# jiangzhengkai/mxdetection

Measured on AMD Instinct MI355X. Metric: images/sec (whole node) Faster R-CNN R50-FPN 3x800x1333, higher is better.
Workload: dtype bf16; 1 GPU; Faster R-CNN ResNet-50-FPN bf16 train step, batch 2/GPU, 3x800x1333 (padded 1344); global_batch=2, parallelism=dp1, frozen=stem+C2, frozen BN folded, optimizer=SGD momentum 0.9 wd 1e-4, launch=hipGraph replay, input=resident, wgrad_side_stream=True, rpn_branch_stream=True, grouped_wgrad=True, filter_prefetch_hints=True, params_trainable=41538304

## Files before the change

### include/mxdet.h

```cpp
#ifndef MXDET_H_
#define MXDET_H_

#include <stddef.h>
#include <stdint.h>

#ifdef __cplusplus
extern "C" {
#endif

#define MXDET_OK 0
#define MXDET_EINVAL (-1)
#define MXDET_ESHAPE (-2)
#define MXDET_EWORKSPACE (-3)
#define MXDET_EHIP (-4)
#define MXDET_ERCCL (-5)

#define MXDET_DTYPE_F32 0
#define MXDET_DTYPE_BF16 1

typedef void* mxdet_stream_t;

const char* mxdet_last_error(void);
const char* mxdet_version(void);

// ... 58 lines not shown
size_t mxdet_atss_assign_workspace_bytes(int32_t N, int64_t A_total, int32_t G_max);
int mxdet_atss_assign(const float* anchors, int64_t A_total, const int64_t* level_offsets , int32_t L,
                      const float* gt_boxes, int32_t N, int32_t G_max, int32_t topk,
                      int32_t* labels, int32_t* matched_gt, float* bbox_targets, float* matched_iou ,
                      void* workspace, size_t workspace_bytes, mxdet_stream_t stream);

int mxdet_proposal_target(const float* rois, const int32_t* num_rois, int32_t rois_stride,
                          const float* gt_boxes, int32_t N, int32_t G_max, int32_t rois_per_image,
                          float fg_fraction, float fg_thresh, float bg_hi, float bg_lo,
                          int32_t num_classes, int32_t class_agnostic,
                          const float* means , const float* stds ,
                          uint32_t seed, uint32_t step, const uint32_t* step_dev,
                          uint32_t image_offset, float* out_rois, int32_t* labels,
                          float* bbox_targets, float* bbox_weights, int32_t* matched_gt,
                          int32_t* num_fg, mxdet_stream_t stream);

int mxdet_fpn_level_map(const float* rois, int64_t R, int32_t lvl_min, int32_t lvl_max,
                        int32_t* levels, mxdet_stream_t stream);
typedef struct {
  int32_t num_levels, lvl_min;
  int32_t H[8], W[8];
  float spatial_scale[8];
  void* feat[8];
} mxdet_feat_pyramid_t;
int mxdet_roi_align_fwd(const mxdet_feat_pyramid_t* f, int32_t N, int32_t C, const float* rois,
                        const int32_t* levels, int64_t R, int32_t PH, int32_t PW,
                        int32_t sampling_ratio, uint16_t* out, mxdet_stream_t stream);
int mxdet_roi_align_bwd(const mxdet_feat_pyramid_t* f, int32_t N, int32_t C, const float* rois,
                        const int32_t* levels, int64_t R, int32_t PH, int32_t PW,
                        int32_t sampling_ratio, const uint16_t* grad_out, mxdet_stream_t stream);
// ... 311 lines not shown
```

### mxdetection_amd/_lib.py

```python
import ctypes as C
import os

_HERE = os.path.dirname(os.path.abspath(__file__))
LIB_PATH = os.environ.get("MXDET_LIB") or os.path.join(_HERE, "libmxdet_hip.so")

c_i32, c_i64, c_u32, c_f32, c_sz, c_vp = C.c_int32, C.c_int64, C.c_uint32, C.c_float, C.c_size_t, C.c_void_p


class PyramidT(C.Structure):
    _fields_ = [
        ("num_levels", c_i32), ("A", c_i32),
        ("H", c_i32 * 8), ("W", c_i32 * 8), ("stride", c_i32 * 8),
        ("cls", c_vp * 8), ("reg", c_vp * 8),
        ("cls_sn", c_i64 * 8), ("cls_sy", c_i64 * 8), ("cls_sx", c_i64 * 8), ("cls_sa", c_i64 * 8),
        ("reg_sn", c_i64 * 8), ("reg_sy", c_i64 * 8), ("reg_sx", c_i64 * 8), ("reg_sc", c_i64 * 8),
        ("dtype", c_i32), ("classes", c_i32),
        ("base_anchors", c_vp * 8),
    ]


class FeatPyramidT(C.Structure):
    _fields_ = [
        ("num_levels", c_i32), ("lvl_min", c_i32),
        ("H", c_i32 * 8), ("W", c_i32 * 8),
# ... 91 lines not shown
    "mxdet_detection_postprocess_soft": (c_i32, [c_vp, c_vp, c_i32, c_i32, c_i32, c_vp, c_vp, c_vp, c_i32, c_i32, c_i32,
                                                 P(c_f32), P(c_f32), c_f32, c_f32, c_i32, c_vp, c_vp, c_vp, c_sz, c_i32,
                                                 c_f32, c_vp]),
    "mxdet_proposal_workspace_bytes": (c_sz, [P(PyramidT), c_i32, c_i32]),
    "mxdet_proposal": (c_i32, [P(PyramidT), c_i32, c_vp, c_i32, c_i32, c_f32, c_f32, c_vp, c_vp, c_vp, c_vp,
                               c_vp, c_sz, c_vp]),
    "mxdet_anchor_target_workspace_bytes": (c_sz, [c_i32, c_i64, c_i32]),
    "mxdet_anchor_target": (c_i32, [c_vp, c_i64, c_vp, c_i32, c_i32, c_vp, c_f32, c_f32, c_f32, c_i32, c_f32,
                                    c_u32, c_u32, c_vp, c_u32, c_vp, c_vp, c_vp, c_vp, c_vp, c_sz, c_vp]),
    "mxdet_atss_assign_workspace_bytes": (c_sz, [c_i32, c_i64, c_i32]),
    "mxdet_atss_assign": (c_i32, [c_vp, c_i64, P(c_i64), c_i32, c_vp, c_i32, c_i32, c_i32, c_vp, c_vp, c_vp, c_vp, c_vp, c_sz,
                                  c_vp]),
    "mxdet_proposal_target": (c_i32, [c_vp, c_vp, c_i32, c_vp, c_i32, c_i32, c_i32, c_f32, c_f32, c_f32, c_f32,
                                      c_i32, c_i32, P(c_f32), P(c_f32), c_u32, c_u32, c_vp, c_u32, c_vp, c_vp, c_vp,
                                      c_vp, c_vp, c_vp, c_vp]),
    "mxdet_fpn_level_map": (c_i32, [c_vp, c_i64, c_i32, c_i32, c_vp, c_vp]),
    "mxdet_roi_align_fwd": (c_i32, [P(FeatPyramidT), c_i32, c_i32, c_vp, c_vp, c_i64, c_i32, c_i32, c_i32, c_vp,
                                    c_vp]),
    "mxdet_roi_align_bwd": (c_i32, [P(FeatPyramidT), c_i32, c_i32, c_vp, c_vp, c_i64, c_i32, c_i32, c_i32, c_vp,
                                    c_vp]),
    "mxdet_roi_align_bwd_gather_workspace_bytes": (c_sz, [P(FeatPyramidT), c_i32, c_i64]),
    "mxdet_roi_align_bwd_gather": (c_i32, [P(FeatPyramidT), c_i32, c_i32, c_vp, c_vp, c_i64, c_i32, c_i32, c_i32, c_vp,
                                           c_i32, c_vp, c_sz, c_vp]),
    "mxdet_roi_align_bwd_gather_prepare": (c_i32, [P(FeatPyramidT), c_i32, c_vp, c_vp, c_i64, c_i32, c_i32, c_i32,
                                                   c_vp, c_sz, c_vp]),
    "mxdet_roi_align_bwd_gather_prepared": (c_i32, [P(FeatPyramidT), c_i32, c_i32, c_vp, c_vp, c_i64, c_i32, c_i32, c_i32,
                                                    c_vp, c_i32, c_vp, c_sz, c_vp]),
    "mxdet_smooth_l1_fwd": (c_i32, [c_vp, c_vp, c_vp, c_i64, c_f32, c_vp, c_vp]),
    "mxdet_smooth_l1_bwd": (c_i32, [c_vp, c_vp, c_vp, c_vp, c_i64, c_f32, c_i32, c_vp, c_vp]),
    "mxdet_loss_workspace_bytes": (c_sz, [c_i64]),
# ... 141 lines not shown
```

### mxdetection_amd/core/bbox.py

```python
import ctypes as C

import torch

from .. import _lib
from .._lib import check, ptr, stream_ptr


def _f32c(t):
    assert t.is_cuda and t.dtype == torch.float32 and t.is_contiguous(), "expected contiguous cuda float32"
    return t


def bbox_overlaps(boxes, query_boxes):
    lib = _lib.load()
    _f32c(boxes), _f32c(query_boxes)
    out = torch.empty((boxes.shape[0], query_boxes.shape[0]), dtype=torch.float32, device=boxes.device)
    check(lib.mxdet_box_iou(ptr(boxes), boxes.shape[0], ptr(query_boxes), query_boxes.shape[0], ptr(out),
                            stream_ptr()), "box_iou")
    return out


def sample_rois(rois, num_rois, gt_boxes, rois_per_image=512, fg_fraction=0.25, fg_thresh=0.5, bg_thresh_hi=0.5,
                bg_thresh_lo=0.0, num_classes=81, class_agnostic=False, bbox_means=(0.0, 0.0, 0.0, 0.0),
                bbox_stds=(0.1, 0.1, 0.2, 0.2), seed=0, step=0, image_offset=0, step_dev=None):
    lib = _lib.load()
    _f32c(rois), _f32c(gt_boxes)
    N, S = rois.shape[0], rois.shape[1]
    G = gt_boxes.shape[1]
    R = rois_per_image
    D = 4 if class_agnostic else 4 * num_classes
    dev = rois.device
    out_rois = torch.empty((N, R, 5), dtype=torch.float32, device=dev)
    labels = torch.empty((N, R), dtype=torch.int32, device=dev)
    tgt = torch.empty((N, R, D), dtype=torch.float32, device=dev)
    wgt = torch.empty((N, R, D), dtype=torch.float32, device=dev)
    matched = torch.empty((N, R), dtype=torch.int32, device=dev)
    num_fg = torch.empty((N,), dtype=torch.int32, device=dev)
    means = (C.c_float * 4)(*bbox_means)
    stds = (C.c_float * 4)(*bbox_stds)
    check(lib.mxdet_proposal_target(ptr(rois), ptr(num_rois), S, ptr(gt_boxes), N, G, R, fg_fraction, fg_thresh,
                                    bg_thresh_hi, bg_thresh_lo, num_classes, int(class_agnostic), means, stds,
                                    seed, step, ptr(step_dev), image_offset, ptr(out_rois), ptr(labels), ptr(tgt), ptr(wgt),
                                    ptr(matched), ptr(num_fg), stream_ptr()), "proposal_target")
    return out_rois, labels, tgt, wgt, matched, num_fg
```

### mxdetection_amd/csrc/boxes.hip

```cpp
#include "common.h"

namespace mxdet {

__global__ void box_iou_kernel(const float4* __restrict__ a, int64_t na, const float4* __restrict__ b,
                               int64_t nb, float* __restrict__ out) {
  int64_t idx = (int64_t)blockIdx.x * blockDim.x + threadIdx.x;
  if (idx >= na * nb) return;
  int64_t i = idx / nb, j = idx - i * nb;
  float4 p = a[i], q = b[j];
  out[idx] = mxdet_iou(p.x, p.y, p.z, p.w, q.x, q.y, q.z, q.w);
}

__global__ void anchors_kernel(const float* __restrict__ base, int A, int H, int W, int stride,
                               float4* __restrict__ out) {
  int64_t idx = (int64_t)blockIdx.x * blockDim.x + threadIdx.x;
  int64_t total = (int64_t)H * W * A;
  if (idx >= total) return;
  int a = (int)(idx % A);
  int64_t cell = idx / A;
  int x = (int)(cell % W), y = (int)(cell / W);
  float sx = (float)(x * stride), sy = (float)(y * stride);
  float4 o;
  o.x = base[a * 4 + 0] + sx;
  o.y = base[a * 4 + 1] + sy;
  o.z = base[a * 4 + 2] + sx;
  o.w = base[a * 4 + 3] + sy;
  out[idx] = o;
}

__global__ void fpn_level_kernel(const float* __restrict__ rois, int64_t R, int lvl_min, int lvl_max,
                                 int32_t* __restrict__ levels) {
  int64_t i = (int64_t)blockIdx.x * blockDim.x + threadIdx.x;
  if (i >= R) return;
  const float* r = rois + i * 5;
  int k = mxdet_fpn_level(r[1], r[2], r[3], r[4]);
  k = k < lvl_min ? lvl_min : (k > lvl_max ? lvl_max : k);
  levels[i] = k;
}

__global__ void __launch_bounds__(64)
nms_mask_kernel(const float4* __restrict__ boxes, const int32_t* __restrict__ counts, int n_max,
                int nwords_max, float thresh, unsigned long long* __restrict__ mask) {
  const int col_blk = blockIdx.x, row_blk = blockIdx.y, b = blockIdx.z;
  if (col_blk < row_blk) return;
  int n = counts[b];
  n = n > n_max ? n_max : n;
  if (row_blk * 64 >= n || col_blk * 64 >= n) return;
  __shared__ float4 cb[64];
  const int t = threadIdx.x;
  const float4* bx = boxes + (int64_t)b * n_max;
  int cj = col_blk * 64 + t;
  if (cj < n) cb[t] = bx[cj];
  __syncthreads();
  int i = row_blk * 64 + t;
  if (i >= n) return;
  float4 r = bx[i];
  int ncol = n - col_blk * 64;
  ncol = ncol > 64 ? 64 : ncol;
  unsigned long long bits = 0;
  for (int j = 0; j < ncol; ++j) {
    int c = col_blk * 64 + j;
    float4 q = cb[j];
    float v = mxdet_iou(r.x, r.y, r.z, r.w, q.x, q.y, q.z, q.w);
    if (c > i && v > thresh) bits |= (1ull << j);
  }
  mask[((int64_t)b * n_max + i) * nwords_max + col_blk] = bits;
}

__device__ __forceinline__ unsigned long long readlane64(unsigned long long v, int lane) {
  unsigned lo = (unsigned)v, hi = (unsigned)(v >> 32);
  lo = (unsigned)__builtin_amdgcn_readlane((int)lo, lane);
  hi = (unsigned)__builtin_amdgcn_readlane((int)hi, lane);
  return ((unsigned long long)hi << 32) | lo;
}

__global__ void __launch_bounds__(64)
nms_scan_kernel(const unsigned long long* __restrict__ mask, const int32_t* __restrict__ counts,
                const uint8_t* __restrict__ invalid, int n_max, int nwords_max, int max_keep,
                int32_t* __restrict__ keep_idx, int32_t* __restrict__ num_keep) {
// ... 47 lines not shown
  }
  int excl = incl - cnt;
  int total = __shfl(incl, 63);
  unsigned long long kb = mykeep;
  int pos = excl;
  while (kb) {
    int bb = __ffsll((long long)kb) - 1;
    kb &= kb - 1;
    if (pos < max_keep) keep_idx[(int64_t)b * n_max + pos] = lane * 64 + bb;
    ++pos;
  }
  if (lane == 0) num_keep[b] = total < max_keep ? total : max_keep;
}

template <int NW>
__global__ void __launch_bounds__(64)
nms_scan_rows_kernel(const unsigned long long* __restrict__ mask, const int32_t* __restrict__ counts,
                     const uint8_t* __restrict__ invalid, int n_max, int nwords_max, int max_keep,
                     int32_t* __restrict__ keep_idx, int32_t* __restrict__ num_keep) {
  __shared__ unsigned long long rows[2][64][NW + 1];
  const int b = blockIdx.x, lane = threadIdx.x;
  int n = counts[b];
  n = n > n_max ? n_max : n;
  n = __builtin_amdgcn_readfirstlane(n);
  const int nw = (n + 63) >> 6;
  const unsigned long long* m = mask + (int64_t)b * n_max * NW;
  unsigned long long myrem = 0ull;
  for (int w = 0; w < nw; ++w) {
    int idx = w * 64 + lane;
    bool bad = (idx >= n) || (invalid != nullptr && invalid[(int64_t)b * n_max + idx] != 0);
    unsigned long long bm = __ballot(bad);
    if (lane == w) myrem = bm;
  }
  unsigned long long nxt[NW];
  auto load_row = [&](unsigned long long (&r)[NW], int w) {
    const unsigned long long* bp = m + (int64_t)(w * 64) * NW + lane;
#pragma unroll
    for (int k = 0; k < NW; ++k) r[k] = bp[k * 64];
  };
  auto stage = [&](const unsigned long long (&r)[NW], int buf, int w) {
    unsigned long long* dst = &rows[buf][lane >> 5][lane & 31];
#pragma unroll
    for (int k = 0; k < NW; ++k) dst[k * 2 * (NW + 1)] = r[k];
  };
  load_row(nxt, 0);
  stage(nxt, 0, 0);
  __syncthreads();
  const int myword = lane < NW ? lane : 0;
  unsigned long long mykeep = 0;
  int buf = 0;
  for (int w = 0; w < nw; ++w) {
#ifndef NMS_ABL_NOLOAD
    if (w + 1 < nw) load_row(nxt, w + 1);
#endif
    const unsigned long long diag = rows[buf][lane][w];
    unsigned long long c = readlane64(myrem, w);
#ifndef NMS_ABL_NOCHAIN
#pragma unroll
    for (int bb = 0; bb < 64; ++bb) {
      unsigned long long d = readlane64(diag, bb);
      c |= ((c >> bb) & 1ull) ? 0ull : d;
    }
#else
    c |= readlane64(diag, 0);
#endif
    const unsigned long long keepbits = ~c;
    if (lane == w) mykeep = keepbits;
    const unsigned klo = __builtin_amdgcn_readfirstlane((unsigned)keepbits);
    const unsigned khi = __builtin_amdgcn_readfirstlane((unsigned)(keepbits >> 32));
    unsigned long long acc = 0ull;
#ifndef NMS_ABL_NOOR
#pragma unroll
#else
    if (klo == 0x12345u)
#endif
    for (int ch = 0; ch < 8; ++ch) {
      const unsigned bits = ((ch < 4 ? klo : khi) >> (8 * (ch & 3))) & 0xffu;
      if (bits == 0u) continue;
      unsigned long long v[8];
#pragma unroll
      for (int t = 0; t < 8; ++t) v[t] = rows[buf][8 * ch + t][myword];
#pragma unroll
      for (int t = 0; t < 8; ++t) acc |= ((bits >> t) & 1u) ? v[t] : 0ull;
    }
    if (lane > w && lane < nw) myrem |= acc;
    if (w + 1 < nw) stage(nxt, buf ^ 1, w + 1);
    __syncthreads();
    buf ^= 1;
  }
  int cnt = __popcll(mykeep);
  int incl = cnt;
  for (int off = 1; off < 64; off <<= 1) {
    int v = __shfl_up(incl, off);
    if (lane >= off) incl += v;
  }
  int excl = incl - cnt;
  int total = __shfl(incl, 63);
  unsigned long long kb = mykeep;
  int pos = excl;
  while (kb) {
    int bb = __ffsll((long long)kb) - 1;
    kb &= kb - 1;
    if (pos < max_keep) keep_idx[(int64_t)b * n_max + pos] = lane * 64 + bb;
    ++pos;
// ... 28 lines not shown
                     as_stream(stream), base_anchors, A, H, W, stride, (float4*)out);
  return check_launch("generate_anchors");
}

extern "C" int mxdet_fpn_level_map(const float* rois, int64_t R, int32_t lvl_min, int32_t lvl_max,
                                   int32_t* levels, mxdet_stream_t stream) {
  clear_error();
  MXDET_REQUIRE(R >= 0 && lvl_min <= lvl_max, MXDET_ESHAPE, "fpn_level_map: bad arguments");
  if (R == 0) return MXDET_OK;
  MXDET_REQUIRE(rois && levels, MXDET_EINVAL, "fpn_level_map: null pointer");
  hipLaunchKernelGGL(fpn_level_kernel, dim3((unsigned)ceil_div<int64_t>(R, 256)), dim3(256), 0,
                     as_stream(stream), rois, R, lvl_min, lvl_max, levels);
  return check_launch("fpn_level_map");
}

extern "C" size_t mxdet_nms_batched_workspace_bytes(int32_t B, int32_t n_max) {
  if (B <= 0 || n_max <= 0) return 0;
  size_t nwords = (size_t)(n_max + 63) / 64;
  if (nwords <= 32) nwords = 32;
  return ((size_t)B * n_max + 64) * nwords * sizeof(unsigned long long);
}

extern "C" int mxdet_nms_batched(const float* boxes, const int32_t* counts, const uint8_t* invalid,
                                 int32_t B, int32_t n_max, float thresh, int32_t max_keep,
                                 int32_t* keep_idx, int32_t* num_keep, void* workspace,
                                 size_t workspace_bytes, mxdet_stream_t stream) {
  clear_error();
  MXDET_REQUIRE(B >= 0 && n_max >= 0, MXDET_ESHAPE, "nms_batched: negative size");
  if (B == 0) return MXDET_OK;
  MXDET_REQUIRE(n_max <= 4096, MXDET_ESHAPE, "nms_batched: n_max %d > 4096 unsupported", n_max);
  MXDET_REQUIRE(counts && num_keep, MXDET_EINVAL, "nms_batched: null pointer");
  if (n_max == 0) {
    hipError_t e = zero_async(num_keep, sizeof(int32_t) * B, as_stream(stream));
    MXDET_REQUIRE(e == hipSuccess, MXDET_EHIP, "nms_batched: memset failed");
    return MXDET_OK;
  }
  MXDET_REQUIRE(boxes && keep_idx, MXDET_EINVAL, "nms_batched: null pointer");
  size_t need = mxdet_nms_batched_workspace_bytes(B, n_max);
  MXDET_REQUIRE(workspace && workspace_bytes >= need, MXDET_EWORKSPACE,
                "nms_batched: workspace %zu < %zu", workspace_bytes, need);
  int nwords = (n_max + 63) / 64;
  const int pitch = nwords <= 32 ? 32 : nwords;
  hipLaunchKernelGGL(nms_mask_kernel, dim3(nwords, nwords, B), dim3(64), 0, as_stream(stream),
                     (const float4*)boxes, counts, n_max, pitch, thresh,
                     (unsigned long long*)workspace);
  if (nwords <= 32)
    hipLaunchKernelGGL(nms_scan_rows_kernel<32>, dim3(B), dim3(64), 0, as_stream(stream),
                       (const unsigned long long*)workspace, counts, invalid, n_max, nwords,
                       max_keep < 0 ? 0 : max_keep, keep_idx, num_keep);
  else
    hipLaunchKernelGGL(nms_scan_kernel, dim3(B), dim3(64), 0, as_stream(stream),
                       (const unsigned long long*)workspace, counts, invalid, n_max, nwords,
                       max_keep < 0 ? 0 : max_keep, keep_idx, num_keep);
  return check_launch("nms_batched");
}
```

### mxdetection_amd/csrc/targets.hip

```cpp
#include "common.h"
#include "select.h"

namespace mxdet {

__global__ void __launch_bounds__(256)
anchor_iou_kernel(const float4* __restrict__ anchors, long long A_total, const float* __restrict__ gt,
                  int G_max, const float* __restrict__ im_info, float allowed_border,
                  float* __restrict__ max_iou, int32_t* __restrict__ argmax,
                  unsigned* __restrict__ gt_max) {
  extern __shared__ __attribute__((aligned(16))) unsigned char smem_raw[];
  float* sg = (float*)smem_raw;
  unsigned* sgm = (unsigned*)(sg + G_max * 5);
  const int n = blockIdx.y;
  for (int i = threadIdx.x; i < G_max * 5; i += blockDim.x) sg[i] = gt[(long long)n * G_max * 5 + i];
  for (int i = threadIdx.x; i < G_max; i += blockDim.x) sgm[i] = 0u;
  __syncthreads();
  long long a = (long long)blockIdx.x * blockDim.x + threadIdx.x;
  if (a < A_total) {
    float4 b = anchors[a];
    float im_h = im_info[n * 3 + 0], im_w = im_info[n * 3 + 1];
    bool inside = (b.x >= -allowed_border) && (b.y >= -allowed_border) &&
                  (b.z < im_w + allowed_border) && (b.w < im_h + allowed_border);
    float best = -1.0f;
    int bi = -1;
// ... 196 lines not shown
    float o[4];
    mxdet_encode(b.x, b.y, b.z, b.w, q[0], q[1], q[2], q[3], o);
    t = make_float4(o[0], o[1], o[2], o[3]);
  }
  targets[idx] = t;
}

__global__ void __launch_bounds__(1024)
proposal_target_kernel(const float* __restrict__ rois, const int32_t* __restrict__ num_rois,
                       int rois_stride, const float* __restrict__ gt, int G_max, int R, int max_fg,
                       float fg_thresh, float bg_hi, float bg_lo, int num_classes, int class_agnostic,
                       float4 means, float4 stds, unsigned seed, unsigned step,
                       const unsigned* __restrict__ step_dev, unsigned image_offset,
                       float* __restrict__ out_rois, int32_t* __restrict__ labels,
                       float* __restrict__ bbox_targets, float* __restrict__ bbox_weights,
                       int32_t* __restrict__ matched_gt, int32_t* __restrict__ num_fg_out) {
  extern __shared__ __attribute__((aligned(16))) unsigned char smem_raw[];
  const int ncap = rois_stride + G_max;
  float* sg = (float*)smem_raw;
  int* vg = (int*)(sg + G_max * 5);
  short* cgt = (short*)(vg + G_max);
  signed char* cstate = (signed char*)(cgt + ((ncap + 7) & ~7));
  __shared__ SelectSmem sm;
  __shared__ int n_valid_gt, cnt_bg;
  const int n = blockIdx.x;
  const unsigned image = image_offset + (unsigned)n;
  if (step_dev) step = *step_dev;
  for (int i = threadIdx.x; i < G_max * 5; i += blockDim.x) sg[i] = gt[(long long)n * G_max * 5 + i];
  if (threadIdx.x == 0) cnt_bg = 0;
  __syncthreads();
  if (threadIdx.x == 0) {
// ... 49 lines not shown
  const int want_bg = (R - nfg) > 0 ? (R - nfg) : 0;
  if (threadIdx.x == 0) cnt_bg = sel_b.n_cand < want_bg ? sel_b.n_cand : want_bg;
  for (int i = threadIdx.x; i < nc; i += blockDim.x) {
    unsigned kv;
    if (cstate[i] == 1) { kfg(i, kv); if (sel_f.chosen(kv, (unsigned)i)) cstate[i] = 3; }
    else if (cstate[i] == 2) { kbg(i, kv); if (sel_b.chosen(kv, (unsigned)i)) cstate[i] = 4; }
  }
  __syncthreads();
  const int nbg = cnt_bg;
  const int reg_dim = class_agnostic ? 4 : 4 * num_classes;
  float* orois = out_rois + (long long)n * R * 5;
  int32_t* olab = labels + (long long)n * R;
  float* otgt = bbox_targets + (long long)n * R * reg_dim;
  float* owgt = bbox_weights + (long long)n * R * reg_dim;
  int32_t* omg = matched_gt + (long long)n * R;
  for (int s = nfg + nbg + threadIdx.x; s < R; s += blockDim.x) {
    float* r = orois + (long long)s * 5;
    r[0] = (float)n; r[1] = 0.f; r[2] = 0.f; r[3] = 0.f; r[4] = 0.f;
    olab[s] = -1;
    omg[s] = -1;
  }
  __syncthreads();
  int base_fg = 0, base_bg = 0;
  for (int base = 0; base < nc; base += blockDim.x) {
    int i = base + threadIdx.x;
    signed char st = (i < nc) ? cstate[i] : 0;
    int tf, tb;
    int rf = block_excl_count(st == 3, sm.scratch, &tf);
    int rbk = block_excl_count(st == 4, sm.scratch, &tb);
    if (st == 3 || st == 4) {
      int slot = (st == 3) ? (base_fg + rf) : (nfg + base_bg + rbk);
      float b[4];
      cand_box(i, b);
      float* r = orois + (long long)slot * 5;
      r[0] = (float)n; r[1] = b[0]; r[2] = b[1]; r[3] = b[2]; r[4] = b[3];
      int g = cgt[i];
      omg[slot] = g;
      if (st == 3) {
        const float* q = sg + g * 5;
        int cls = (int)q[4];
        olab[slot] = cls;
        float o[4];
        mxdet_encode(b[0], b[1], b[2], b[3], q[0], q[1], q[2], q[3], o);
        int c0 = class_agnostic ? 0 : 4 * cls;
        float* t = otgt + (long long)slot * reg_dim + c0;
        float* w = owgt + (long long)slot * reg_dim + c0;
        t[0] = (o[0] - means.x) / stds.x;
        t[1] = (o[1] - means.y) / stds.y;
        t[2] = (o[2] - means.z) / stds.z;
        t[3] = (o[3] - means.w) / stds.w;
// ... 81 lines not shown
  hipLaunchKernelGGL(anchor_nogt_kernel, grid, dim3(256), 0, s, (const float4*)anchors,
                     (long long)A_total, gt_boxes, G_max, im_info, allowed_border, seed, step, step_dev,
                     image_offset, labels, miou, w.keys, cl);
  if (batch_size > 0) {
    int max_fg = (int)(fg_fraction * (float)batch_size);
    hipLaunchKernelGGL(anchor_sample_kernel, dim3(N), dim3(1024), 0, s, (long long)A_total,
                       batch_size, max_fg, (const int32_t*)labels, (const unsigned*)w.keys, cl, w.sel);
  }
  hipLaunchKernelGGL(anchor_encode_kernel, grid, dim3(256), 0, s, (const float4*)anchors,
                     (long long)A_total, gt_boxes, G_max, labels, amax, (const unsigned*)w.keys,
                     batch_size > 0 ? (const AnchorSel*)w.sel : (const AnchorSel*)nullptr,
                     (float4*)bbox_targets);
  return check_launch("anchor_target");
}

extern "C" int mxdet_proposal_target(const float* rois, const int32_t* num_rois, int32_t rois_stride,
                                     const float* gt_boxes, int32_t N, int32_t G_max,
                                     int32_t rois_per_image, float fg_fraction, float fg_thresh,
                                     float bg_hi, float bg_lo, int32_t num_classes,
                                     int32_t class_agnostic, const float* means, const float* stds,
                                     uint32_t seed, uint32_t step, const uint32_t* step_dev,
                                     uint32_t image_offset, float* out_rois, int32_t* labels,
                                     float* bbox_targets,
                                     float* bbox_weights, int32_t* matched_gt, int32_t* num_fg,
                                     mxdet_stream_t stream) {
  clear_error();
  MXDET_REQUIRE(N > 0 && rois_stride > 0 && G_max > 0 && rois_per_image > 0 && num_classes > 0,
                MXDET_ESHAPE, "proposal_target: bad sizes");
  MXDET_REQUIRE(rois && num_rois && gt_boxes && means && stds && out_rois && labels && bbox_targets &&
                    bbox_weights && matched_gt && num_fg,
                MXDET_EINVAL, "proposal_target: null pointer");
  MXDET_REQUIRE(G_max <= 1024 && rois_stride <= 16384, MXDET_ESHAPE, "proposal_target: too large");
  int ncap = rois_stride + G_max;
  size_t lds = (size_t)G_max * 5 * 4 + (size_t)G_max * 4 + (size_t)((ncap + 7) & ~7) * 2 +
               (size_t)((ncap + 15) & ~15);
  MXDET_REQUIRE(lds <= 120 * 1024, MXDET_ESHAPE, "proposal_target: LDS budget exceeded");
  int max_fg = (int)(fg_fraction * (float)rois_per_image);
  float4 m = make_float4(means[0], means[1], means[2], means[3]);
  float4 sd = make_float4(stds[0], stds[1], stds[2], stds[3]);
  {
    const size_t reg_dim = class_agnostic ? 4 : 4 * (size_t)num_classes;
    const size_t bytes = (size_t)N * rois_per_image * reg_dim * sizeof(float);
    hipError_t e = zero_async(bbox_targets, bytes, as_stream(stream));
    if (e == hipSuccess) e = zero_async(bbox_weights, bytes, as_stream(stream));
    MXDET_REQUIRE(e == hipSuccess, MXDET_EHIP, "proposal_target: zero fill failed");
  }
  hipLaunchKernelGGL(proposal_target_kernel, dim3(N), dim3(1024), lds, as_stream(stream), rois,
                     num_rois, rois_stride, gt_boxes, G_max, rois_per_image, max_fg, fg_thresh, bg_hi,
                     bg_lo, num_classes, class_agnostic, m, sd, seed, step, step_dev, image_offset, out_rois,
                     labels, bbox_targets, bbox_weights, matched_gt, num_fg);
  return check_launch("proposal_target");
}
```

### mxdetection_amd/models/bbox_heads/convfc_bbox_head.py

```python
import os

import torch

from ...core import bbox as B_
from ...core import loss as L_
from ...ops import dense
from ..utils.layers import ConvLayer, GroupNormLayer, cached_buf


class BBoxHead:
    def __init__(self, in_features, arena, ws, device, gen, num_classes=81, fc_dim=1024, rois_per_image=512,
                 fg_fraction=0.25, fg_thresh=0.5, bg_hi=0.5, bg_lo=0.0, stds=(0.1, 0.1, 0.2, 0.2), sigma=1.0,
                 seed=99, reg_loss="smooth_l1", reg_loss_weight=1.0):
        L_.check_reg_loss(reg_loss, reg_loss_weight)
        self.reg_loss, self.reg_loss_weight = reg_loss, float(reg_loss_weight)
        kw = dict(arena=arena, ws=ws, device=device, gen=gen)
        self.nc = num_classes
        self.reg_dim = 4 * num_classes
        self.ld = (num_classes + self.reg_dim + 63) // 64 * 64
        self.fc_out = ConvLayer("bbox.fc_out", fc_dim, self.ld, 1, init_std=0.01, cout_real=num_classes + self.reg_dim, **kw)
        self._build_trunk(in_features, fc_dim, kw)
        self.fc_out.fc_in_hwc = ()
        self.R, self.fg_fraction, self.fg_thresh, self.bg_hi, self.bg_lo = rois_per_image, fg_fraction, fg_thresh, bg_hi, bg_lo
        self.stds, self.sigma, self.seed, self.device = stds, sigma, seed, device
# ... 13 lines not shown

    def norm_layers(self):
        return []

    def _buf(self, key, shape, dtype=torch.bfloat16, zero=False):
        return cached_buf(self.bufs, key, shape, dtype, self.device, zero)

    def plan(self, N):
        R = N * self.R
        self.fc1.plan((R, 1, 1, self.in_features))
        self.fc2.plan((R, 1, 1, self.fc_dim))
        self.fc_out.plan((R, 1, 1, self.fc_dim))
        self.loss = torch.zeros((2,), dtype=torch.float32, device=self.device)
        self.loss_ws = L_.loss_workspace(R, self.device)

    def sample(self, rois, num_rois, gt_boxes, step, image_offset, step_dev=None):
        out = B_.sample_rois(rois, num_rois, gt_boxes, self.R, self.fg_fraction, self.fg_thresh, self.bg_hi, self.bg_lo,
                             self.nc, False, (0.0, 0.0, 0.0, 0.0), self.stds, self.seed, step, image_offset, step_dev)
        self.rois, self.labels, self.tgt, self.wgt, self.matched, self.num_fg = out
        self.gt_boxes = gt_boxes
        return self.rois.view(-1, 5)

    def forward(self, pooled):
        R = pooled.shape[0]
        self.x = pooled.view(R, 1, 1, -1)
        ks = self.fc1_ksplit if (R * self.fc_dim) % (64 * 64 * 8) == 0 and R % 64 == 0 else 1
        if ks > 1:
            need = 4 * ks * R * self.fc_dim
            ws = self._buf("fc1_ws", (need,), dtype=torch.uint8)
            self.h1 = dense.conv2d_forward_splitk(self.x, self.fc1.w_bf16, self.fc1.bias_f32, None, True, ks,
                                                  self._buf("h1", (R, 1, 1, self.fc_dim)), ws)
        else:
            self.h1 = self.fc1.forward(self.x, relu=True, out=self._buf("h1", (R, 1, 1, self.fc_dim)))
        self.h2 = self.fc2.forward(self.h1, relu=True, out=self._buf("h2", (R, 1, 1, self.fc_dim)))
# ... 102 lines not shown
```

### mxdetection_amd/models/faster_rcnn.py

```python
import torch

from ..core.loss import check_reg_loss
from .backbones import ResNet
from .bbox_heads import BBoxHead, ConvFCBBoxHead
from .mask_heads import FCNMaskHead
from .necks import FPN
from .roi_extractors import DeformRoIExtractor, FPNRoIExtractor
from .rpn_heads import RPNHead
from .utils.detector import DetectorBase
from .utils.layers import Workspace


def check_head_options(bbox_head, head_norm, gn_groups, with_mask):
    if bbox_head not in ("2fc", "4conv1fc"):
        raise ValueError("bbox_head must be '2fc' or '4conv1fc' (got %r)" % (bbox_head,))
    if head_norm not in ("none", "gn"):
        raise ValueError("head_norm must be 'none' or 'gn' (got %r)" % (head_norm,))
    if head_norm == "gn":
        if bbox_head == "2fc" and not with_mask:
            raise ValueError("head_norm='gn' with nothing to normalise: the 2fc box head has no convolutions and there "
                             "is no mask head")
        g = gn_groups
        if not isinstance(g, int) or isinstance(g, bool) or g <= 0 or 256 % g or (256 // g) % 8:
            raise ValueError("gn_groups = %r does not divide 256 channels into groups of a multiple of 8" % (g,))
# ... 82 lines not shown
        N, _, H, W = image.shape
        self.plan(N, H, W, gt_boxes.shape[1])
        early = self.branch is not None
        if early:
            with self._branch_ctx():
                self.rpn_head.assign_targets(gt_boxes, im_info, step, image_offset, step_dev)
        C = self.backbone.forward(image)
        P = self.neck.forward(C)
        self.rpn_head.forward(P)
        defer_rpn = (self.roi_bwd_gather and self.ws.side is not None and self.ws_rpn.grouping and self.ws.grouping
                     and self._bucket_here(0))
        with self._branch_ctx():
            rpn_loss = self.rpn_head.loss_and_grad(gt_boxes, im_info, step, image_offset, step_dev=step_dev, assigned=early)
            self.rpn_head.backward(self.dP, [False] * 5, flush=not defer_rpn)
        rois, _, _, num_rois = self.rpn_head.get_proposals(im_info)
        rois_s = self.bbox_head.sample(rois, num_rois, gt_boxes, step, image_offset, step_dev)
        pooled = self.roi_extractor.forward(P, rois_s, prepare_gather=self.roi_bwd_gather)
        self.bbox_head.forward(pooled)
        rcnn_loss = self.bbox_head.loss_and_grad()
        mask_loss = None
        if self.with_mask:
            mrois = self.mask_head.select_rois(self.bbox_head)
            self.mask_head.targets(gt_masks)
            mpooled = self.mask_roi_extractor.forward(P, mrois, prepare_gather=self.roi_bwd_gather)
            self.mask_head.forward(mpooled)
            mask_loss = self.mask_head.loss_and_grad()
        if self.with_mask:
            d_mpooled = self.mask_head.backward()
        d_pooled = self.bbox_head.backward()
        if self.roi_bwd_gather:
            self._join_branch()
            lo = 0
# ... 56 lines not shown
```

### mxdetection_amd/models/roi_extractors/fpn_roi_extractor.py

```python
import torch

from ...ops import dense
from ...ops.roi_align import (fpn_level_map, roi_align_backward, roi_align_backward_gather,
                              roi_align_backward_gather_prepare, roi_align_backward_gather_workspace, roi_align_forward)


class FPNRoIExtractor:
    def __init__(self, strides, pooled=(7, 7), sampling_ratio=2, lvl_min=2, device="cuda"):
        self.scales = [1.0 / s for s in strides]
        self.pooled, self.sr, self.lvl_min = pooled, sampling_ratio, lvl_min
        self.lvl_max = lvl_min + len(strides) - 1
        self.device = device
        self.out = None
        self.outs = {}
        self.dacc = None
        self.gather_ws = {}
        self.prepared = None

    def forward(self, feats, rois, prepare_gather=False):
        self.feats, self.rois = feats[:len(self.scales)], rois
        self.levels = fpn_level_map(rois, self.lvl_min, self.lvl_max)
        R, C = rois.shape[0], feats[0].shape[3]
        self.out = self.outs.setdefault((R, C), None)
        if self.out is None:
            self.out = torch.empty((R, self.pooled[0], self.pooled[1], C), dtype=torch.bfloat16, device=self.device)
            self.outs[(R, C)] = self.out
        self.prepared = None
        if prepare_gather:
            key = (R,) + tuple(tuple(f.shape[:3]) for f in self.feats)
            ws = self.gather_ws.get(key)
            if ws is None:
                ws = self.gather_ws[key] = roi_align_backward_gather_workspace(self.feats, self.scales, R, self.lvl_min)
            roi_align_backward_gather_prepare(self.feats, self.scales, rois, self.levels, self.pooled, self.sr,
                                              self.lvl_min, ws)
            self.prepared = ws
        return roi_align_forward(self.feats, self.scales, rois, self.levels, self.pooled, self.sr, self.lvl_min, self.out)
# ... 37 lines not shown
```

### mxdetection_amd/ops/nms.py

```python
import torch

from .. import _lib
from .._lib import check, ptr, stream_ptr


def nms_batched(boxes, counts, thresh, max_keep=None, invalid=None):
    lib = _lib.load()
    B, n = boxes.shape[0], boxes.shape[1]
    dev = boxes.device
    keep = torch.full((B, max(n, 1)), -1, dtype=torch.int32, device=dev)
    num = torch.zeros((B,), dtype=torch.int32, device=dev)
    ws_bytes = lib.mxdet_nms_batched_workspace_bytes(B, n)
    ws = torch.empty((max(ws_bytes, 8),), dtype=torch.uint8, device=dev)
    check(lib.mxdet_nms_batched(ptr(boxes), ptr(counts), ptr(invalid), B, n, thresh,
                                n if max_keep is None else max_keep, ptr(keep), ptr(num), ptr(ws), ws_bytes,
                                stream_ptr()), "nms_batched")
    return keep, num


SOFT_NMS_METHODS = {"hard": 0, "linear": 1, "gaussian": 2}


def soft_nms_method(name):
    if name not in SOFT_NMS_METHODS:
        raise ValueError("nms_method %r: expected one of %s" % (name, sorted(SOFT_NMS_METHODS)))
    return SOFT_NMS_METHODS[name]


# ... 12 lines not shown
```

Baseline: 480.0 images/sec.

## Restructure batched NMS mask/scan kernels and fuse FPN level mapping into ROI sampling

The NMS mask kernel now launches only the upper-triangular block pairs, packing four column blocks per 256-thread workgroup, and also records within-block column suppression bits. The row-scan kernel becomes a 256-thread kernel that resolves each 64-box word with an iterative ballot fixed point, spreads the OR-reduction over four waves and prefetches three words ahead. Separately, proposal-target sampling now also writes FPN level indices, so the ROI extractor no longer launches its own level-map kernel. nms_batched also accepts a caller-supplied workspace. These changes aim to cut kernel count and serial latency in the RPN/ROI stage, but add more complex synchronisation and a fixed-point loop that can take up to 64 rounds.

```diff
diff --git a/include/mxdet.h b/include/mxdet.h
--- a/include/mxdet.h
+++ b/include/mxdet.h
@@ -96,6 +96,16 @@
                           uint32_t image_offset, float* out_rois, int32_t* labels,
                           float* bbox_targets, float* bbox_weights, int32_t* matched_gt,
                           int32_t* num_fg, mxdet_stream_t stream);
+int mxdet_proposal_target_levels(const float* rois, const int32_t* num_rois, int32_t rois_stride,
+                                 const float* gt_boxes, int32_t N, int32_t G_max, int32_t rois_per_image,
+                                 float fg_fraction, float fg_thresh, float bg_hi, float bg_lo,
+                                 int32_t num_classes, int32_t class_agnostic,
+                                 const float* means , const float* stds ,
+                                 uint32_t seed, uint32_t step, const uint32_t* step_dev,
+                                 uint32_t image_offset, float* out_rois, int32_t* labels,
+                                 float* bbox_targets, float* bbox_weights, int32_t* matched_gt,
+                                 int32_t* num_fg, int32_t lvl_min, int32_t lvl_max, int32_t* levels,
+                                 mxdet_stream_t stream);
 
 int mxdet_fpn_level_map(const float* rois, int64_t R, int32_t lvl_min, int32_t lvl_max,
                         int32_t* levels, mxdet_stream_t stream);
diff --git a/mxdetection_amd/_lib.py b/mxdetection_amd/_lib.py
--- a/mxdetection_amd/_lib.py
+++ b/mxdetection_amd/_lib.py
@@ -129,6 +129,9 @@
     "mxdet_proposal_target": (c_i32, [c_vp, c_vp, c_i32, c_vp, c_i32, c_i32, c_i32, c_f32, c_f32, c_f32, c_f32,
                                       c_i32, c_i32, P(c_f32), P(c_f32), c_u32, c_u32, c_vp, c_u32, c_vp, c_vp, c_vp,
                                       c_vp, c_vp, c_vp, c_vp]),
+    "mxdet_proposal_target_levels": (c_i32, [c_vp, c_vp, c_i32, c_vp, c_i32, c_i32, c_i32, c_f32, c_f32, c_f32, c_f32,
+                                             c_i32, c_i32, P(c_f32), P(c_f32), c_u32, c_u32, c_vp, c_u32, c_vp, c_vp, c_vp,
+                                             c_vp, c_vp, c_vp, c_i32, c_i32, c_vp, c_vp]),
     "mxdet_fpn_level_map": (c_i32, [c_vp, c_i64, c_i32, c_i32, c_vp, c_vp]),
     "mxdet_roi_align_fwd": (c_i32, [P(FeatPyramidT), c_i32, c_i32, c_vp, c_vp, c_i64, c_i32, c_i32, c_i32, c_vp,
                                     c_vp]),
diff --git a/mxdetection_amd/core/bbox.py b/mxdetection_amd/core/bbox.py
--- a/mxdetection_amd/core/bbox.py
+++ b/mxdetection_amd/core/bbox.py
@@ -22,7 +22,7 @@
 
 def sample_rois(rois, num_rois, gt_boxes, rois_per_image=512, fg_fraction=0.25, fg_thresh=0.5, bg_thresh_hi=0.5,
                 bg_thresh_lo=0.0, num_classes=81, class_agnostic=False, bbox_means=(0.0, 0.0, 0.0, 0.0),
-                bbox_stds=(0.1, 0.1, 0.2, 0.2), seed=0, step=0, image_offset=0, step_dev=None):
+                bbox_stds=(0.1, 0.1, 0.2, 0.2), seed=0, step=0, image_offset=0, step_dev=None, fpn_levels=None):
     lib = _lib.load()
     _f32c(rois), _f32c(gt_boxes)
     N, S = rois.shape[0], rois.shape[1]
@@ -38,8 +38,13 @@
     num_fg = torch.empty((N,), dtype=torch.int32, device=dev)
     means = (C.c_float * 4)(*bbox_means)
     stds = (C.c_float * 4)(*bbox_stds)
-    check(lib.mxdet_proposal_target(ptr(rois), ptr(num_rois), S, ptr(gt_boxes), N, G, R, fg_fraction, fg_thresh,
-                                    bg_thresh_hi, bg_thresh_lo, num_classes, int(class_agnostic), means, stds,
-                                    seed, step, ptr(step_dev), image_offset, ptr(out_rois), ptr(labels), ptr(tgt), ptr(wgt),
-                                    ptr(matched), ptr(num_fg), stream_ptr()), "proposal_target")
-    return out_rois, labels, tgt, wgt, matched, num_fg
+    args = (ptr(rois), ptr(num_rois), S, ptr(gt_boxes), N, G, R, fg_fraction, fg_thresh, bg_thresh_hi, bg_thresh_lo,
+            num_classes, int(class_agnostic), means, stds, seed, step, ptr(step_dev), image_offset, ptr(out_rois),
+            ptr(labels), ptr(tgt), ptr(wgt), ptr(matched), ptr(num_fg))
+    if fpn_levels is None:
+        check(lib.mxdet_proposal_target(*args, stream_ptr()), "proposal_target")
+        return out_rois, labels, tgt, wgt, matched, num_fg
+    levels = torch.empty((N, R), dtype=torch.int32, device=dev)
+    check(lib.mxdet_proposal_target_levels(*args, fpn_levels[0], fpn_levels[1], ptr(levels), stream_ptr()),
+          "proposal_target_levels")
+    return out_rois, labels, tgt, wgt, matched, num_fg, levels
diff --git a/mxdetection_amd/csrc/boxes.hip b/mxdetection_amd/csrc/boxes.hip
--- a/mxdetection_amd/csrc/boxes.hip
+++ b/mxdetection_amd/csrc/boxes.hip
@@ -38,31 +38,51 @@
   levels[i] = k;
 }
 
-__global__ void __launch_bounds__(64)
-nms_mask_kernel(const float4* __restrict__ boxes, const int32_t* __restrict__ counts, int n_max,
-                int nwords_max, float thresh, unsigned long long* __restrict__ mask) {
-  const int col_blk = blockIdx.x, row_blk = blockIdx.y, b = blockIdx.z;
-  if (col_blk < row_blk) return;
+__global__ void __launch_bounds__(256)
+nms_mask_kernel(const float4* __restrict__ boxes, const int32_t* __restrict__ counts, int n_max, int nwords,
+                int nwords_max, float thresh, unsigned long long* __restrict__ mask,
+                unsigned long long* __restrict__ cols) {
+  __shared__ float4 cb[4][64];
+  const int b = blockIdx.y, wave = threadIdx.x >> 6, t = threadIdx.x & 63;
+  int row_blk = 0, rest = blockIdx.x;
+  for (int r = 0; r < nwords; ++r) {
+    const int groups = (nwords - r + 3) >> 2;
+    if (rest < groups) { row_blk = r; break; }
+    rest -= groups;
+  }
+  const int col_blk = row_blk + rest * 4 + wave;
   int n = counts[b];
   n = n > n_max ? n_max : n;
-  if (row_blk * 64 >= n || col_blk * 64 >= n) return;
-  __shared__ float4 cb[64];
-  const int t = threadIdx.x;
+  if (row_blk * 64 >= n) return;
+  const bool live = col_blk < nwords && col_blk * 64 < n;
   const float4* bx = boxes + (int64_t)b * n_max;
   int cj = col_blk * 64 + t;
-  if (cj < n) cb[t] = bx[cj];
+  cb[wave][t] = (live && cj < n) ? bx[cj] : make_float4(0.f, 0.f, 0.f, 0.f);
   __syncthreads();
   int i = row_blk * 64 + t;
-  if (i >= n) return;
+  if (!live || i >= n) return;
   float4 r = bx[i];
   int ncol = n - col_blk * 64;
   ncol = ncol > 64 ? 64 : ncol;
   unsigned long long bits = 0;
-  for (int j = 0; j < ncol; ++j) {
-    int c = col_blk * 64 + j;
-    float4 q = cb[j];
-    float v = mxdet_iou(r.x, r.y, r.z, r.w, q.x, q.y, q.z, q.w);
-    if (c > i && v > thresh) bits |= (1ull << j);
+  if (col_blk != row_blk) {
+    for (int j = 0; j < ncol; ++j) {
+      float4 q = cb[wave][j];
+      float v = mxdet_iou(r.x, r.y, r.z, r.w, q.x, q.y, q.z, q.w);
+      if (v > thresh) bits |= (1ull << j);
+    }
+  } else {
+    unsigned long long cbits = 0;
+    for (int j = 0; j < ncol; ++j) {
+      float4 q = cb[wave][j];
+      const bool up = j > t;
+      float4 p0 = up ? r : q, p1 = up ? q : r;
+      float v = mxdet_iou(p0.x, p0.y, p0.z, p0.w, p1.x, p1.y, p1.z, p1.w);
+      if (j != t && v > thresh) {
+        if (up) bits |= (1ull << j); else cbits |= (1ull << j);
+      }
+    }
+    cols[(int64_t)b * n_max + i] = cbits;
   }
   mask[((int64_t)b * n_max + i) * nwords_max + col_blk] = bits;
 }
@@ -140,80 +160,109 @@
 }
 
 template <int NW>
-__global__ void __launch_bounds__(64)
-nms_scan_rows_kernel(const unsigned long long* __restrict__ mask, const int32_t* __restrict__ counts,
-                     const uint8_t* __restrict__ invalid, int n_max, int nwords_max, int max_keep,
+__global__ void __launch_bounds__(256)
+nms_scan_rows_kernel(const unsigned long long* __restrict__ mask, const unsigned long long* __restrict__ cols,
+                     const int32_t* __restrict__ counts, const uint8_t* __restrict__ invalid, int n_max, int max_keep,
                      int32_t* __restrict__ keep_idx, int32_t* __restrict__ num_keep) {
+  static_assert(NW == 32, "the thread -> (row group, word) maps below assume 32 words");
+  constexpr int kGroups = 256 / NW;
+  constexpr int kRowsPer = 64 / kGroups;
+  constexpr int kLoads = 64 * NW / 256;
   __shared__ unsigned long long rows[2][64][NW + 1];
-  const int b = blockIdx.x, lane = threadIdx.x;
+  __shared__ unsigned long long part[2][kGroups][NW];
+  __shared__ unsigned long long rem0[NW];
+  __shared__ unsigned long long colw[2][64];
+  const int b = blockIdx.x, tid = threadIdx.x, lane = tid & 63, wave = tid >> 6;
   int n = counts[b];
   n = n > n_max ? n_max : n;
   n = __builtin_amdgcn_readfirstlane(n);
   const int nw = (n + 63) >> 6;
   const unsigned long long* m = mask + (int64_t)b * n_max * NW;
-  unsigned long long myrem = 0ull;
-  for (int w = 0; w < nw; ++w) {
-    int idx = w * 64 + lane;
-    bool bad = (idx >= n) || (invalid != nullptr && invalid[(int64_t)b * n_max + idx] != 0);
-    unsigned long long bm = __ballot(bad);
-    if (lane == w) myrem = bm;
-  }
-  unsigned long long nxt[NW];
-  auto load_row = [&](unsigned long long (&r)[NW], int w) {
-    const unsigned long long* bp = m + (int64_t)(w * 64) * NW + lane;
-#pragma unroll
-    for (int k = 0; k < NW; ++k) r[k] = bp[k * 64];
+  const unsigned long long* cl = cols + (int64_t)b * n_max;
+  {
+    bool bad[NW / 4];
+#pragma unroll
+    for (int k = 0; k < NW / 4; ++k) {
+      int idx = (wave + 4 * k) * 64 + lane;
+      bad[k] = (idx >= n) || (invalid != nullptr && invalid[(int64_t)b * n_max + idx] != 0);
+    }
+#pragma unroll
+    for (int k = 0; k < NW / 4; ++k) {
+      unsigned long long bm = __ballot(bad[k]);
+      if (lane == 0) rem0[wave + 4 * k] = bm;
+    }
+  }
+  struct Fetch { unsigned long long r[kLoads], col; };
+  auto load_rows = [&](Fetch& f, int w) {
+    if (w >= nw) return;
+    const unsigned long long* bp = m + (int64_t)(w * 64) * NW + tid;
+#pragma unroll
+    for (int k = 0; k < kLoads; ++k) f.r[k] = bp[k * 256];
+    const int idx = w * 64 + lane;
+    f.col = idx < n ? cl[idx] : 0ull;
   };
-  auto stage = [&](const unsigned long long (&r)[NW], int buf, int w) {
-    unsigned long long* dst = &rows[buf][lane >> 5][lane & 31];
-#pragma unroll
-    for (int k = 0; k < NW; ++k) dst[k * 2 * (NW + 1)] = r[k];
+  auto stage = [&](const Fetch& f, int buf) {
+    unsigned long long* dst = &rows[buf][tid / NW][tid % NW];
+#pragma unroll
+    for (int k = 0; k < kLoads; ++k) dst[k * kGroups * (NW + 1)] = f.r[k];
+    if (wave == 0) colw[buf][lane] = f.col;
   };
-  load_row(nxt, 0);
-  stage(nxt, 0, 0);
+  Fetch fa, fb, fc;
+  load_rows(fa, 0);
+  load_rows(fb, 1);
+  load_rows(fc, 2);
+  if (nw > 0) stage(fa, 0);
   __syncthreads();
-  const int myword = lane < NW ? lane : 0;
+  const int myword = lane % NW;
+  const int grp = tid / NW;
+  unsigned long long myrem = rem0[myword];
   unsigned long long mykeep = 0;
-  int buf = 0;
-  for (int w = 0; w < nw; ++w) {
+  auto word = [&](int w, Fetch& ld, const Fetch& st) {
+    const int buf = w & 1;
 #ifndef NMS_ABL_NOLOAD
-    if (w + 1 < nw) load_row(nxt, w + 1);
+    load_rows(ld, w + 3);
 #endif
-    const unsigned long long diag = rows[buf][lane][w];
-    unsigned long long c = readlane64(myrem, w);
+    const unsigned long long col = colw[buf][lane];
+    const unsigned long long removed = readlane64(myrem, w);
+    const bool alive = !((removed >> lane) & 1ull);
+    unsigned long long K = ~removed;
 #ifndef NMS_ABL_NOCHAIN
-#pragma unroll
-    for (int bb = 0; bb < 64; ++bb) {
-      unsigned long long d = readlane64(diag, bb);
-      c |= ((c >> bb) & 1ull) ? 0ull : d;
+    for (int round = 0; round < 64; ++round) {
+      const unsigned long long K1 = __ballot(alive && (col & K) == 0ull);
+      if (K1 == K) break;
+      K = K1;
     }
 #else
-    c |= readlane64(diag, 0);
+    K = __ballot(alive && (col & K) == 0ull);
 #endif
-    const unsigned long long keepbits = ~c;
+    const unsigned long long keepbits = K;
     if (lane == w) mykeep = keepbits;
-    const unsigned klo = __builtin_amdgcn_readfirstlane((unsigned)keepbits);
-    const unsigned khi = __builtin_amdgcn_readfirstlane((unsigned)(keepbits >> 32));
     unsigned long long acc = 0ull;
-#ifndef NMS_ABL_NOOR
-#pragma unroll
-#else
-    if (klo == 0x12345u)
+#ifdef NMS_ABL_NOOR
+    if (keepbits == 0x12345ull)
 #endif
-    for (int ch = 0; ch < 8; ++ch) {
-      const unsigned bits = ((ch < 4 ? klo : khi) >> (8 * (ch & 3))) & 0xffu;
-      if (bits == 0u) continue;
-      unsigned long long v[8];
-#pragma unroll
-      for (int t = 0; t < 8; ++t) v[t] = rows[buf][8 * ch + t][myword];
-#pragma unroll
-      for (int t = 0; t < 8; ++t) acc |= ((bits >> t) & 1u) ? v[t] : 0ull;
-    }
-    if (lane > w && lane < nw) myrem |= acc;
-    if (w + 1 < nw) stage(nxt, buf ^ 1, w + 1);
+    {
+      const unsigned kb = (unsigned)(keepbits >> (kRowsPer * grp)) & ((1u << kRowsPer) - 1u);
+      unsigned long long v[kRowsPer];
+#pragma unroll
+      for (int t = 0; t < kRowsPer; ++t) v[t] = rows[buf][kRowsPer * grp + t][myword];
+#pragma unroll
+      for (int t = 0; t < kRowsPer; ++t) acc |= ((kb >> t) & 1u) ? v[t] : 0ull;
+    }
+    part[buf][grp][myword] = acc;
+    if (w + 1 < nw) stage(st, buf ^ 1);
     __syncthreads();
-    buf ^= 1;
-  }
+    unsigned long long sum = 0ull;
+#pragma unroll
+    for (int g = 0; g < kGroups; ++g) sum |= part[buf][g][myword];
+    if (myword > w && myword < nw) myrem |= sum;
+  };
+  for (int w = 0; w < nw; w += 3) {
+    word(w, fa, fb);
+    if (w + 1 < nw) word(w + 1, fb, fc);
+    if (w + 2 < nw) word(w + 2, fc, fa);
+  }
+  if (wave != 0) return;
   int cnt = __popcll(mykeep);
   int incl = cnt;
   for (int off = 1; off < 64; off <<= 1) {
@@ -272,11 +321,15 @@
   return check_launch("fpn_level_map");
 }
 
-extern "C" size_t mxdet_nms_batched_workspace_bytes(int32_t B, int32_t n_max) {
-  if (B <= 0 || n_max <= 0) return 0;
+static size_t nms_mask_bytes(int32_t B, int32_t n_max) {
   size_t nwords = (size_t)(n_max + 63) / 64;
   if (nwords <= 32) nwords = 32;
   return ((size_t)B * n_max + 64) * nwords * sizeof(unsigned long long);
+}
+
+extern "C" size_t mxdet_nms_batched_workspace_bytes(int32_t B, int32_t n_max) {
+  if (B <= 0 || n_max <= 0) return 0;
+  return nms_mask_bytes(B, n_max) + (size_t)B * n_max * sizeof(unsigned long long);
 }
 
 extern "C" int mxdet_nms_batched(const float* boxes, const int32_t* counts, const uint8_t* invalid,
@@ -299,12 +352,15 @@
                 "nms_batched: workspace %zu < %zu", workspace_bytes, need);
   int nwords = (n_max + 63) / 64;
   const int pitch = nwords <= 32 ? 32 : nwords;
-  hipLaunchKernelGGL(nms_mask_kernel, dim3(nwords, nwords, B), dim3(64), 0, as_stream(stream),
-                     (const float4*)boxes, counts, n_max, pitch, thresh,
-                     (unsigned long long*)workspace);
+  unsigned long long* cols = (unsigned long long*)((char*)workspace + nms_mask_bytes(B, n_max));
+  int tri = 0;
+  for (int r = 0; r < nwords; ++r) tri += (nwords - r + 3) / 4;
+  hipLaunchKernelGGL(nms_mask_kernel, dim3(tri, B), dim3(256), 0, as_stream(stream),
+                     (const float4*)boxes, counts, n_max, nwords, pitch, thresh,
+                     (unsigned long long*)workspace, cols);
   if (nwords <= 32)
-    hipLaunchKernelGGL(nms_scan_rows_kernel<32>, dim3(B), dim3(64), 0, as_stream(stream),
-                       (const unsigned long long*)workspace, counts, invalid, n_max, nwords,
+    hipLaunchKernelGGL(nms_scan_rows_kernel<32>, dim3(B), dim3(256), 0, as_stream(stream),
+                       (const unsigned long long*)workspace, (const unsigned long long*)cols, counts, invalid, n_max,
                        max_keep < 0 ? 0 : max_keep, keep_idx, num_keep);
   else
     hipLaunchKernelGGL(nms_scan_kernel, dim3(B), dim3(64), 0, as_stream(stream),
diff --git a/mxdetection_amd/csrc/targets.hip b/mxdetection_amd/csrc/targets.hip
--- a/mxdetection_amd/csrc/targets.hip
+++ b/mxdetection_amd/csrc/targets.hip
@@ -234,7 +234,8 @@
                        const unsigned* __restrict__ step_dev, unsigned image_offset,
                        float* __restrict__ out_rois, int32_t* __restrict__ labels,
                        float* __restrict__ bbox_targets, float* __restrict__ bbox_weights,
-                       int32_t* __restrict__ matched_gt, int32_t* __restrict__ num_fg_out) {
+                       int32_t* __restrict__ matched_gt, int32_t* __restrict__ num_fg_out, int lvl_min, int lvl_max,
+                       int32_t* __restrict__ levels) {
   extern __shared__ __attribute__((aligned(16))) unsigned char smem_raw[];
   const int ncap = rois_stride + G_max;
   float* sg = (float*)smem_raw;
@@ -314,11 +315,17 @@
   float* otgt = bbox_targets + (long long)n * R * reg_dim;
   float* owgt = bbox_weights + (long long)n * R * reg_dim;
   int32_t* omg = matched_gt + (long long)n * R;
+  int32_t* olvl = levels ? levels + (long long)n * R : nullptr;
+  auto fpn_lvl = [&](float x1, float y1, float x2, float y2) {
+    int k = mxdet_fpn_level(x1, y1, x2, y2);
+    return k < lvl_min ? lvl_min : (k > lvl_max ? lvl_max : k);
+  };
   for (int s = nfg + nbg + threadIdx.x; s < R; s += blockDim.x) {
     float* r = orois + (long long)s * 5;
     r[0] = (float)n; r[1] = 0.f; r[2] = 0.f; r[3] = 0.f; r[4] = 0.f;
     olab[s] = -1;
     omg[s] = -1;
+    if (olvl) olvl[s] = fpn_lvl(0.f, 0.f, 0.f, 0.f);
   }
   __syncthreads();
   int base_fg = 0, base_bg = 0;
@@ -334,6 +341,7 @@
       cand_box(i, b);
       float* r = orois + (long long)slot * 5;
       r[0] = (float)n; r[1] = b[0]; r[2] = b[1]; r[3] = b[2]; r[4] = b[3];
+      if (olvl) olvl[slot] = fpn_lvl(b[0], b[1], b[2], b[3]);
       int g = cgt[i];
       omg[slot] = g;
       if (st == 3) {
@@ -445,16 +453,16 @@
   return check_launch("anchor_target");
 }
 
-extern "C" int mxdet_proposal_target(const float* rois, const int32_t* num_rois, int32_t rois_stride,
-                                     const float* gt_boxes, int32_t N, int32_t G_max,
-                                     int32_t rois_per_image, float fg_fraction, float fg_thresh,
-                                     float bg_hi, float bg_lo, int32_t num_classes,
-                                     int32_t class_agnostic, const float* means, const float* stds,
-                                     uint32_t seed, uint32_t step, const uint32_t* step_dev,
-                                     uint32_t image_offset, float* out_rois, int32_t* labels,
-                                     float* bbox_targets,
-                                     float* bbox_weights, int32_t* matched_gt, int32_t* num_fg,
-                                     mxdet_stream_t stream) {
+static int proposal_target_impl(const float* rois, const int32_t* num_rois, int32_t rois_stride,
+                                const float* gt_boxes, int32_t N, int32_t G_max,
+                                int32_t rois_per_image, float fg_fraction, float fg_thresh,
+                                float bg_hi, float bg_lo, int32_t num_classes,
+                                int32_t class_agnostic, const float* means, const float* stds,
+                                uint32_t seed, uint32_t step, const uint32_t* step_dev,
+                                uint32_t image_offset, float* out_rois, int32_t* labels,
+                                float* bbox_targets,
+                                float* bbox_weights, int32_t* matched_gt, int32_t* num_fg,
+                                int32_t lvl_min, int32_t lvl_max, int32_t* levels, mxdet_stream_t stream) {
   clear_error();
   MXDET_REQUIRE(N > 0 && rois_stride > 0 && G_max > 0 && rois_per_image > 0 && num_classes > 0,
                 MXDET_ESHAPE, "proposal_target: bad sizes");
@@ -479,6 +487,40 @@
   hipLaunchKernelGGL(proposal_target_kernel, dim3(N), dim3(1024), lds, as_stream(stream), rois,
                      num_rois, rois_stride, gt_boxes, G_max, rois_per_image, max_fg, fg_thresh, bg_hi,
                      bg_lo, num_classes, class_agnostic, m, sd, seed, step, step_dev, image_offset, out_rois,
-                     labels, bbox_targets, bbox_weights, matched_gt, num_fg);
+                     labels, bbox_targets, bbox_weights, matched_gt, num_fg, lvl_min, lvl_max, levels);
   return check_launch("proposal_target");
 }
+
+extern "C" int mxdet_proposal_target(const float* rois, const int32_t* num_rois, int32_t rois_stride,
+                                     const float* gt_boxes, int32_t N, int32_t G_max,
+                                     int32_t rois_per_image, float fg_fraction, float fg_thresh,
+                                     float bg_hi, float bg_lo, int32_t num_classes,
+                                     int32_t class_agnostic, const float* means, const float* stds,
+                                     uint32_t seed, uint32_t step, const uint32_t* step_dev,
+                                     uint32_t image_offset, float* out_rois, int32_t* labels,
+                                     float* bbox_targets,
+                                     float* bbox_weights, int32_t* matched_gt, int32_t* num_fg,
+                                     mxdet_stream_t stream) {
+  return proposal_target_impl(rois, num_rois, rois_stride, gt_boxes, N, G_max, rois_per_image, fg_fraction, fg_thresh,
+                              bg_hi, bg_lo, num_classes, class_agnostic, means, stds, seed, step, step_dev, image_offset,
+                              out_rois, labels, bbox_targets, bbox_weights, matched_gt, num_fg, 0, 0, nullptr, stream);
+}
+
+extern "C" int mxdet_proposal_target_levels(const float* rois, const int32_t* num_rois, int32_t rois_stride,
+                                            const float* gt_boxes, int32_t N, int32_t G_max,
+                                            int32_t rois_per_image, float fg_fraction, float fg_thresh,
+                                            float bg_hi, float bg_lo, int32_t num_classes,
+                                            int32_t class_agnostic, const float* means, const float* stds,
+                                            uint32_t seed, uint32_t step, const uint32_t* step_dev,
+                                            uint32_t image_offset, float* out_rois, int32_t* labels,
+                                            float* bbox_targets, float* bbox_weights, int32_t* matched_gt,
+                                            int32_t* num_fg, int32_t lvl_min, int32_t lvl_max, int32_t* levels,
+                                            mxdet_stream_t stream) {
+  clear_error();
+  MXDET_REQUIRE(levels != nullptr, MXDET_EINVAL, "proposal_target_levels: null levels");
+  MXDET_REQUIRE(lvl_min <= lvl_max, MXDET_ESHAPE, "proposal_target_levels: lvl_min %d > lvl_max %d", lvl_min, lvl_max);
+  return proposal_target_impl(rois, num_rois, rois_stride, gt_boxes, N, G_max, rois_per_image, fg_fraction, fg_thresh,
+                              bg_hi, bg_lo, num_classes, class_agnostic, means, stds, seed, step, step_dev, image_offset,
+                              out_rois, labels, bbox_targets, bbox_weights, matched_gt, num_fg, lvl_min, lvl_max, levels,
+                              stream);
+}
diff --git a/mxdetection_amd/models/bbox_heads/convfc_bbox_head.py b/mxdetection_amd/models/bbox_heads/convfc_bbox_head.py
--- a/mxdetection_amd/models/bbox_heads/convfc_bbox_head.py
+++ b/mxdetection_amd/models/bbox_heads/convfc_bbox_head.py
@@ -51,10 +51,12 @@
         self.loss = torch.zeros((2,), dtype=torch.float32, device=self.device)
         self.loss_ws = L_.loss_workspace(R, self.device)
 
-    def sample(self, rois, num_rois, gt_boxes, step, image_offset, step_dev=None):
+    def sample(self, rois, num_rois, gt_boxes, step, image_offset, step_dev=None, fpn_levels=None):
         out = B_.sample_rois(rois, num_rois, gt_boxes, self.R, self.fg_fraction, self.fg_thresh, self.bg_hi, self.bg_lo,
-                             self.nc, False, (0.0, 0.0, 0.0, 0.0), self.stds, self.seed, step, image_offset, step_dev)
-        self.rois, self.labels, self.tgt, self.wgt, self.matched, self.num_fg = out
+                             self.nc, False, (0.0, 0.0, 0.0, 0.0), self.stds, self.seed, step, image_offset, step_dev,
+                             fpn_levels=fpn_levels)
+        self.rois, self.labels, self.tgt, self.wgt, self.matched, self.num_fg = out[:6]
+        self.roi_levels = out[6].view(-1) if fpn_levels is not None else None
         self.gt_boxes = gt_boxes
         return self.rois.view(-1, 5)
 
diff --git a/mxdetection_amd/models/faster_rcnn.py b/mxdetection_amd/models/faster_rcnn.py
--- a/mxdetection_amd/models/faster_rcnn.py
+++ b/mxdetection_amd/models/faster_rcnn.py
@@ -120,8 +120,14 @@
             rpn_loss = self.rpn_head.loss_and_grad(gt_boxes, im_info, step, image_offset, step_dev=step_dev, assigned=early)
             self.rpn_head.backward(self.dP, [False] * 5, flush=not defer_rpn)
         rois, _, _, num_rois = self.rpn_head.get_proposals(im_info)
-        rois_s = self.bbox_head.sample(rois, num_rois, gt_boxes, step, image_offset, step_dev)
-        pooled = self.roi_extractor.forward(P, rois_s, prepare_gather=self.roi_bwd_gather)
+        if self.dpool is None:
+            ext = self.roi_extractor
+            rois_s = self.bbox_head.sample(rois, num_rois, gt_boxes, step, image_offset, step_dev,
+                                           fpn_levels=(ext.lvl_min, ext.lvl_max))
+            pooled = ext.forward(P, rois_s, prepare_gather=self.roi_bwd_gather, levels=self.bbox_head.roi_levels)
+        else:
+            rois_s = self.bbox_head.sample(rois, num_rois, gt_boxes, step, image_offset, step_dev)
+            pooled = self.roi_extractor.forward(P, rois_s, prepare_gather=self.roi_bwd_gather)
         self.bbox_head.forward(pooled)
         rcnn_loss = self.bbox_head.loss_and_grad()
         mask_loss = None
diff --git a/mxdetection_amd/models/roi_extractors/fpn_roi_extractor.py b/mxdetection_amd/models/roi_extractors/fpn_roi_extractor.py
--- a/mxdetection_amd/models/roi_extractors/fpn_roi_extractor.py
+++ b/mxdetection_amd/models/roi_extractors/fpn_roi_extractor.py
@@ -17,9 +17,9 @@
         self.gather_ws = {}
         self.prepared = None
 
-    def forward(self, feats, rois, prepare_gather=False):
+    def forward(self, feats, rois, prepare_gather=False, levels=None):
         self.feats, self.rois = feats[:len(self.scales)], rois
-        self.levels = fpn_level_map(rois, self.lvl_min, self.lvl_max)
+        self.levels = levels if levels is not None else fpn_level_map(rois, self.lvl_min, self.lvl_max)
         R, C = rois.shape[0], feats[0].shape[3]
         self.out = self.outs.setdefault((R, C), None)
         if self.out is None:
diff --git a/mxdetection_amd/ops/nms.py b/mxdetection_amd/ops/nms.py
--- a/mxdetection_amd/ops/nms.py
+++ b/mxdetection_amd/ops/nms.py
@@ -4,14 +4,15 @@
 from .._lib import check, ptr, stream_ptr
 
 
-def nms_batched(boxes, counts, thresh, max_keep=None, invalid=None):
+def nms_batched(boxes, counts, thresh, max_keep=None, invalid=None, workspace=None):
     lib = _lib.load()
     B, n = boxes.shape[0], boxes.shape[1]
     dev = boxes.device
     keep = torch.full((B, max(n, 1)), -1, dtype=torch.int32, device=dev)
     num = torch.zeros((B,), dtype=torch.int32, device=dev)
     ws_bytes = lib.mxdet_nms_batched_workspace_bytes(B, n)
-    ws = torch.empty((max(ws_bytes, 8),), dtype=torch.uint8, device=dev)
+    ws = workspace if workspace is not None else torch.empty((max(ws_bytes, 8),), dtype=torch.uint8, device=dev)
+    ws_bytes = ws.numel() if workspace is not None else ws_bytes
     check(lib.mxdet_nms_batched(ptr(boxes), ptr(counts), ptr(invalid), B, n, thresh,
                                 n if max_keep is None else max_keep, ptr(keep), ptr(num), ptr(ws), ws_bytes,
                                 stream_ptr()), "nms_batched")
```

Measured after the change: 479.5 images/sec. About the same (-0.1%).
